# jontio/JAERO

Hardware: AMD Instinct MI355X
Metric: Msamples/s of real 48 kHz PCM through the 10.5 kbps OQPSK demodulator hot path (higher is better)
Workload: dtype f64; 1 GPU; 65536-channel-per-GPU synthetic 48 kHz 10.5 kbps OQPSK continuous (BASELINE configs[2] shape, scaled to 65536 channels per GPU = one wavefront of 64 channels per SIMD), 4096-sample writes, coarse 2^14 FFT every 4096 samples, AFC off, EbNo meters on, Eb/N0 10.0 dB, per-channel carrier (8000 +- 100 Hz), bits, noise, symbol phase; 42 untimed pre-roll steps (the last 18 resident and back to back with ; channels_per_gpu=65536, total_channels=65536, chunk=4096, ebno_meters=True, preroll_steps=42, timing_phases=32, hbm_bytes_per_resident_channel=2256640, resident_channels_max=137027, ranks=1, control_plane=none (single rank), sustain_steps=18

## Files before the change

jaero_amd/csrc/k_burst_front.h:

```cpp
#pragma once
#include "burst_device.h"
#include "jaero_device.h"
#include "k_coarse2.h"
#include "k_coarse6.h"
#include "k_pre8400.h"

#define BLDF(f) (p.S[(size_t)(f) * nchp + ch])
#define BLDI(f) (p.I[(size_t)(f) * nchp + ch])

__device__ __forceinline__ size_t hb_idx(int slot, int nchp, int ch) { return ((size_t)(slot >> 2) * nchp + ch) * 4 + (slot & 3); }
__global__ __launch_bounds__(PF_THREADS) void k_hilbert_fft(const BGeom g, const BPtrs p, int ns, long long n0)
{
    extern __shared__ double hf_xch[];
    const int tid = threadIdx.x, c = tid & 3, T = tid >> 2;
    const int nchp = g.nchp, H = g.hist_len;
    const int cha = blockIdx.x * 8 + 2 * c;
    const long long m0 = ((n0 >> 11) + blockIdx.y) << 11;
    const int i0 = (int)(m0 - n0);
    const int16_t *__restrict__ hist = p.pcmhist;
    CV<16> d;
    {
        const long long tb = m0 - g.hil_lat - 2048 + T + 4LL * H;
#pragma unroll
        for (int s = 0; s < 16; s++)
        {
            const int slot = (int)((tb + 256 * s) % H);
            const size_t o = hb_idx(slot, nchp, cha);
            d.r[s] = (double)hist[o];
            d.i[s] = (double)hist[o + 4];
        }
    }
    pf_fft4096(d, hf_xch, p.tw12, T, c);
    {
        const double2 *__restrict__ Hh = p.hilH + T;
#pragma unroll
        for (int s = 0; s < 16; s++)
        {
            const double2 h = Hh[256 * s];
            const double yr = d.r[s] * h.x - d.i[s] * h.y, yi = d.r[s] * h.y + d.i[s] * h.x;
            d.r[s] = yr; d.i[s] = -yi;
        }
    }
    pf_fft4096(d, hf_xch, p.tw12, T, c);
    const int grp = cha >> 6, lane = cha & 63;
#pragma unroll
    for (int s = 8; s < 16; s++)
    {
        const int i = i0 + T + 256 * (s - 8);
        if (i >= 0 && i < ns)
        {
            const size_t q = ((size_t)grp * g.maxseg + i) * 64 + lane;
            *(double2 *)(p.him + q) = make_double2(d.r[s] / 32768.0, (-d.i[s]) / 32768.0);
        }
    }
}

__global__ void k_hist_push_frames(const int16_t *__restrict__ src, int stride, int nch, int16_t *__restrict__ hist, int nchp, int H,
                                   int slot0, int n)
{
    const int c = blockIdx.x * blockDim.x + threadIdx.x;
    const int i = blockIdx.y;
    if (c >= nchp || i >= n) return;
    int slot = slot0 + i; if (slot >= H) slot -= H;
    hist[hb_idx(slot, nchp, c)] = (c < nch) ? src[(size_t)i * stride + c] : (int16_t)0;
}
__global__ void k_hist_push_chmajor(const int16_t *__restrict__ src, int nch, int n, int16_t *__restrict__ hist, int nchp, int H, int slot0)
{
    __shared__ int16_t tile[64][65];
    const int c0 = blockIdx.x * 64, i0 = blockIdx.y * 64;
    const int tx = threadIdx.x & 63, ty = threadIdx.x >> 6;
    for (int r = ty; r < 64; r += 4)
    {
        const int c = c0 + r, i = i0 + tx;
        tile[r][tx] = (c < nch && i < n) ? src[(size_t)c * n + i] : (int16_t)0;
    }
    __syncthreads();
    for (int r = ty; r < 64; r += 4)
    {
        const int i = i0 + r, c = c0 + tx;
        if (i < n && c < nchp)
        {
            int slot = (slot0 + i) % H;
            hist[hb_idx(slot, nchp, c)] = tile[tx][r];
        }
    }
}

#define FB 8
__device__ __forceinline__ int bwrap(int s, int len) { return s >= len ? s - len : s; }
__device__ __forceinline__ int bback(int s, int lag, int len) { s -= lag; return s < 0 ? s + len : s; }

template <bool HOLD>
__global__ __launch_bounds__(64) void k_burst_front(const BGeom g, const BPtrs p, int n, long long n0)
{
    const int lane = threadIdx.x, grp = blockIdx.x, ch = grp * 64 + lane, nchp = g.nchp;
    double agc_sum = BLDF(BS_AGC_SUM), ma1_re = BLDF(BS_MA1_RE), ma1_im = BLDF(BS_MA1_IM), mav1_sum = BLDF(BS_MAV1_SUM), lastdy = BLDF(BS_LASTDY);
    int cntdown = BLDI(BI_CNTDOWN), maxposcd = BLDI(BI_MAXPOSCD), tri_ptr = BLDI(BI_TRI_PTR);
    const int flags = BLDI(BI_FLAGS);
    int ev_pos = -1, ev_cnt = BLDI(BI_EV_CNT);
    int hold = HOLD ? BLDI(BI_BT_HOLD) : 0;
    const bool trace = (g.flags & 8u) != 0;

    const double *__restrict__ him = p.him + (size_t)grp * g.maxseg * 64 + lane;
    const int16_t *__restrict__ hist = p.pcmhist;
    const int s_re0 = (int)((n0 - g.hil_lat - 1024 + 4LL * g.hist_len) % g.hist_len);
    double *agc_ring = p.agc_ring + (size_t)grp * g.agc_len * 64 + lane;
    double *cvre = p.cvre + (size_t)grp * g.cv_len * 64 + lane;
    double *cvim = p.cvim + (size_t)grp * g.cv_len * 64 + lane;
    double *ma1r = p.ma1re + (size_t)grp * g.ma1_len * 64 + lane;
    double *ma1i = p.ma1im + (size_t)grp * g.ma1_len * 64 + lane;
    double *mav1 = p.mav1 + (size_t)grp * g.mav1_len * 64 + lane;
    double *fa = p.fa + (size_t)grp * g.fa_len * 64 + lane;
    double *bt = p.bt + (size_t)grp * g.bt_len * 64 + lane;

    int s_agc = (int)(n0 % g.agc_len), s_cv = (int)(n0 % g.cv_len), s_ma1 = (int)(n0 % g.ma1_len), s_mav1 = (int)(n0 % g.mav1_len);
    int s_fa = (int)(n0 % g.fa_len), s_bt = (int)(n0 % g.bt_len);
    const double agc_len_d = (double)g.agc_len, ma1_len_d = (double)g.ma1_len, mav1_len_d = (double)g.mav1_len;
    const double btw = g.bt_w, btwc = 1.0 - g.bt_w, faw = g.fa_w, fawc = 1.0 - g.fa_w;
    const int twoPL = 2 * g.PL;

    for (int i0 = 0; i0 < n; i0 += FB)
    {
        double x_re[FB], x_im[FB], o_agc[FB], o_m1r[FB], o_m1i[FB], o_mav[FB], fa_old[FB], fa_new[FB], bt_2[FB], bt_1[FB];
        double co_r[FB], co_i[FB], cn_r[FB], cn_i[FB];
#pragma unroll
        for (int k = 0; k < FB; k++)
        {
            const int ii = (i0 + k < n) ? i0 + k : n - 1;
            const int d = ii - i0;
            x_re[k] = -(((double)hist[hb_idx(bwrap(s_re0 + ii, g.hist_len), nchp, ch)]) / 32768.0); x_im[k] = him[(size_t)ii * 64];
            o_agc[k] = agc_ring[(size_t)bwrap(s_agc + d, g.agc_len) * 64];
            o_m1r[k] = ma1r[(size_t)bwrap(s_ma1 + d, g.ma1_len) * 64];
            o_m1i[k] = ma1i[(size_t)bwrap(s_ma1 + d, g.ma1_len) * 64];
            o_mav[k] = mav1[(size_t)bwrap(s_mav1 + d, g.mav1_len) * 64];
            const int cs = bwrap(s_cv + d, g.cv_len);
            const int c_old = bback(cs, g.bt_lag, g.cv_len), c_new = bwrap(c_old + 1, g.cv_len);
            co_r[k] = cvre[(size_t)c_old * 64]; co_i[k] = cvim[(size_t)c_old * 64];
            cn_r[k] = cvre[(size_t)c_new * 64]; cn_i[k] = cvim[(size_t)c_new * 64];
            const int fs = bwrap(s_fa + d, g.fa_len);
            const int f_old = bback(fs, g.fa_lag, g.fa_len), f_new = bwrap(f_old + 1, g.fa_len);
            fa_old[k] = fa[(size_t)f_old * 64]; fa_new[k] = fa[(size_t)f_new * 64];
            const int bs = bwrap(s_bt + d, g.bt_len);
            bt_2[k] = bt[(size_t)bback(bs, twoPL, g.bt_len) * 64];
            bt_1[k] = bt[(size_t)bback(bs, g.PL, g.bt_len) * 64];
        }
#pragma unroll
        for (int k = 0; k < FB; k++)
        {
            const int i = i0 + k;
            if (i >= n) break;
            const double a = hypot(x_re[k], x_im[k]);
            agc_sum = agc_sum - o_agc[k];
            agc_sum = agc_sum + fabs(a);
            agc_ring[(size_t)s_agc * 64] = fabs(a);
            double gain = 1.414213562 / fmax(agc_sum / agc_len_d, 0.000001);
            gain = fmax(gain, 0.000001);
            const double c_re = x_re[k] * gain, c_im = x_im[k] * gain;
            cvre[(size_t)s_cv * 64] = c_re; cvim[(size_t)s_cv * 64] = c_im;
            double nr = cn_r[k], ni = cn_i[k], orr = co_r[k], oi = co_i[k];
            if (g.bt_lag == 1) { nr = c_re; ni = c_im; }
            if (HOLD)
            {
                if (hold > 0) { orr = 0.0; oi = 0.0; }
                if (hold > 1) { nr = 0.0; ni = 0.0; }
                if (hold > 0) hold--;
            }
            const double dl_re = btw * nr + btwc * orr, dl_im = btw * ni + btwc * oi;
            const double pr = c_re * dl_re - c_im * (-dl_im), pi = c_re * (-dl_im) + c_im * dl_re;
            ma1_re = ma1_re - o_m1r[k]; ma1_im = ma1_im - o_m1i[k];
            ma1_re = ma1_re + pr; ma1_im = ma1_im + pi;
            ma1r[(size_t)s_ma1 * 64] = pr; ma1i[(size_t)s_ma1 * 64] = pi;
            double fastarm = hypot(ma1_re / ma1_len_d, ma1_im / ma1_len_d);
            mav1_sum = mav1_sum - o_mav[k];
            mav1_sum = mav1_sum + fastarm;
            mav1[(size_t)s_mav1 * 64] = fastarm;
            fastarm = mav1_sum / mav1_len_d;
            fa[(size_t)s_fa * 64] = fastarm;
            fastarm -= (faw * fa_new[k] + fawc * fa_old[k]);
            if (fastarm < 0) fastarm = 0;
            double bt_sig = fastarm * fastarm;
            if (bt_sig > 500) bt_sig = 500;
            bt[(size_t)s_bt * 64] = bt_sig;
            const double dy = bt_sig - bt_2[k];
            const double vald = bt_1[k];
            const bool trig = (!cntdown) && (vald > g.pd_thr) && (lastdy >= 0 && dy < 0);
            unsigned long long tm = __ballot(trig);
            if (tm)
            {
                const int pos0 = bback(s_bt, twoPL, g.bt_len);
                const double *btg = p.bt + (size_t)grp * g.bt_len * 64;
                __builtin_amdgcn_fence(__ATOMIC_RELEASE, "wavefront");
                __builtin_amdgcn_s_waitcnt(0x0f70);
                while (tm)
                {
                    const int src = __ffsll((long long)tm) - 1;
                    tm &= tm - 1;
                    double bv = 0.0;
                    int bq = -1;
                    for (int q = lane; q <= twoPL; q += 64)
                    {
                        const double v = btg[(size_t)bwrap(pos0 + q, g.bt_len) * 64 + src];
                        if (bq < 0 || v > bv) { bv = v; bq = q; }
                    }
#pragma unroll
                    for (int off = 32; off > 0; off >>= 1)
                    {
                        const double ov = __shfl_xor(bv, off, 64);
                        const int oq = __shfl_xor(bq, off, 64);
                        if (oq >= 0 && (bq < 0 || ov > bv || (ov == bv && oq < bq))) { bv = ov; bq = oq; }
                    }
                    if (lane == src) { cntdown = twoPL; maxposcd = bq; }
                }
            }
            if (cntdown > 0) cntdown--;
            lastdy = dy;
            bool fire = false;
            if (!maxposcd) { maxposcd--; fire = true; }
            else if (maxposcd > 0) maxposcd--;
            if (fire)
            {
                tri_ptr = 0;
                if (trace && ev_cnt < g.ev_cap)
                {
                    double *e = p.evlog + ((size_t)ch * g.ev_cap + ev_cnt) * 3;
                    e[0] = (double)(n0 + i); e[1] = BEV_PEAK; e[2] = 0; ev_cnt++;
                }
            }
            if (tri_ptr < g.tri_sz) tri_ptr++;
            else if (tri_ptr == g.tri_sz) { tri_ptr++; ev_pos = i; }
            s_agc = bwrap(s_agc + 1, g.agc_len); s_cv = bwrap(s_cv + 1, g.cv_len); s_ma1 = bwrap(s_ma1 + 1, g.ma1_len);
            s_mav1 = bwrap(s_mav1 + 1, g.mav1_len); s_fa = bwrap(s_fa + 1, g.fa_len); s_bt = bwrap(s_bt + 1, g.bt_len);
        }
    }
    BLDF(BS_AGC_SUM) = agc_sum; BLDF(BS_MA1_RE) = ma1_re; BLDF(BS_MA1_IM) = ma1_im; BLDF(BS_MAV1_SUM) = mav1_sum; BLDF(BS_LASTDY) = lastdy;
    BLDI(BI_CNTDOWN) = cntdown; BLDI(BI_MAXPOSCD) = maxposcd; BLDI(BI_TRI_PTR) = tri_ptr; BLDI(BI_EV_POS) = ev_pos; BLDI(BI_EV_CNT) = ev_cnt;
    (void)flags;
    if (HOLD) BLDI(BI_BT_HOLD) = hold;
    const unsigned long long em = __ballot(ev_pos >= 0 && ch < g.nch);
    if (lane == 0) p.ev_mask[grp] = em;
}

__global__ __launch_bounds__(1024) void k_ev_compact(const unsigned long long *__restrict__ mask, int ngroups, int *__restrict__ ev_list, int *__restrict__ ev_count)
{
    __shared__ int part[1024];
    const int t = threadIdx.x;
    const int per = (ngroups + 1023) / 1024;
    const int g0 = t * per, g1 = (g0 + per < ngroups) ? g0 + per : ngroups;
    int cnt = 0;
    for (int gq = g0; gq < g1; gq++) cnt += __popcll(mask[gq]);
    part[t] = cnt;
    __syncthreads();
    for (int off = 1; off < 1024; off <<= 1)
    {
        const int v = (t >= off) ? part[t - off] : 0;
        __syncthreads();
        part[t] += v;
        __syncthreads();
    }
    int base = part[t] - cnt;
    for (int gq = g0; gq < g1; gq++)
    {
        unsigned long long m = mask[gq];
        while (m)
        {
            const int ln = __ffsll((long long)m) - 1;
            m &= m - 1;
            ev_list[base++] = gq * 64 + ln;
        }
    }
    if (t == 1023) *ev_count = part[1023];
}

#define TRI_N 32768
#define TRI_H 16384

template <int NTHREADS>
__device__ __forceinline__ void tri_argmax_first(double &v, int &idx, double *red_val, int *red_idx, int t)
{
#pragma unroll
    for (int off = 32; off > 0; off >>= 1)
    {
        const double ov = __shfl_xor(v, off, 64);
        const int oi = __shfl_xor(idx, off, 64);
        if (oi >= 0 && (idx < 0 || ov > v || (ov == v && oi < idx))) { v = ov; idx = oi; }
    }
    __syncthreads();
    if ((t & 63) == 0) { red_val[t >> 6] = v; red_idx[t >> 6] = idx; }
    __syncthreads();
    v = red_val[0]; idx = red_idx[0];
#pragma unroll
    for (int w = 1; w < NTHREADS / 64; w++)
    {
        const double ov = red_val[w];
        const int oi = red_idx[w];
        if (oi >= 0 && (idx < 0 || ov > v || (ov == v && oi < idx))) { v = ov; idx = oi; }
    }
}

#define TRI_THREADS 256
#define TRI_XCH C6_XCH13
template <bool oq>
__global__ __launch_bounds__(TRI_THREADS, 2) void k_trident(const BGeom g, const BPtrs p, long long n0)
{
    extern __shared__ __attribute__((aligned(16))) double xch[];
    __shared__ double red_val[TRI_THREADS / 64];
    __shared__ int red_idx[TRI_THREADS / 64];
    __shared__ double sh_bb[2];
    double *dl = xch;
    const int t = threadIdx.x, nchp = g.nchp;
    const int nev = *p.ev_count;
    const double hzperbin = g.Fs / ((double)TRI_N);
    const int b = jd_qround((0.25 * g.fb) / hzperbin), b4 = b >> 2;
    const int psb = jd_qround((0.5 * g.fb) / hzperbin);
    const int nx = gridDim.x < 8 ? 1 : 8;
    const int xcd = blockIdx.x % nx, wx = blockIdx.x / nx, nwx = (gridDim.x + nx - 1 - xcd) / nx;
    const int e_lo = (int)(((long long)nev * xcd) / nx), e_hi = (int)(((long long)nev * (xcd + 1)) / nx);
    for (int li = e_lo + wx; li < e_hi; li += nwx)
    {
        const int ch = p.ev_list[li];
        const int grp = ch >> 6, lane = ch & 63;
        const int evp = p.I[(size_t)BI_EV_POS * nchp + ch];
        const long long w0 = n0 + evp - g.tri_sz - g.D1 + 8LL * g.cv_len;
        const double *__restrict__ cvre = p.cvre + (size_t)grp * g.cv_len * 64 + lane;
        double mag[16];
        double bv = -1.0, bre = 0.0, bim = 0.0;
        int bi = -1;
        double minval = 0.0;
        int minvalbin = 0;
        double mv = 0.0; int mi = -1;
        double lv = 0.0; int lidx = -1;
        double hv = 0.0; int hidx = -1;
        for (int pass = 0; pass < 8; pass++)
        {
            const int which = oq ? (pass & 1) : (pass >> 2), r = oq ? (pass >> 1) : (pass & 3);
            const int off = which ? g.nb : 0, len = which ? g.nt : g.nb;
            if (!oq && pass == 4)
            {
                minval = bv; minvalbin = bi;
                tri_argmax_first<TRI_THREADS>(minval, minvalbin, red_val, red_idx, t);
                if (bi == minvalbin) { sh_bb[0] = bre; sh_bb[1] = bim; }
                if (!(minval > 0.0)) minvalbin = 0;
            }
            CV<32> d;
            const int slot0 = (int)((w0 + off) % g.cv_len);
#pragma unroll
            for (int s = 0; s < 32; s++)
            {
                const int n = s * TRI_THREADS + t;
                if (s * TRI_THREADS >= len) { d.r[s] = 0.0; d.i[s] = 0.0; continue; }
                double x0 = 0.0, x1 = 0.0;
                if (n < len)
                {
                    int sl = slot0 + n; if (sl >= g.cv_len) sl -= g.cv_len;
                    x0 = cvre[(size_t)sl * 64];
                }
                if (len > 8192 && n + 8192 < len)
                {
                    int sl = slot0 + n + 8192; while (sl >= g.cv_len) sl -= g.cv_len;
                    x1 = cvre[(size_t)sl * 64];
                }
                double fr = x0, fi = 0.0;
                if (r == 0) fr += x1; else if (r == 1) fi -= x1; else if (r == 2) fr -= x1; else fi += x1;
                if (r == 0) { d.r[s] = fr; d.i[s] = fi; }
                else
                {
                    const int m = n * r;
                    double2 w = p.tw15[m & (TRI_H - 1)];
                    if (m & TRI_H) { w.x = -w.x; w.y = -w.y; }
                    d.r[s] = fr * w.x - fi * w.y; d.i[s] = fr * w.y + fi * w.x;
                }
            }
            wg_fft13_e32(d, xch, p.tw14, t);
            if (which == 0)
            {
#pragma unroll
                for (int s = 0; s < 16; s++)
                {
                    const int k = 4 * (s * TRI_THREADS + t) + r;
                    const double a = hypot(d.r[s], d.i[s]);
                    mag[s] = a;
                    if (a > bv || (a == bv && k < bi)) { bv = a; bi = k; bre = d.r[s]; bim = d.i[s]; }
                }
            }
            else if (oq)
            {
                __syncthreads();
#pragma unroll
                for (int s = 0; s < 16; s++) dl[s * TRI_THREADS + t] = hypot(d.r[s], d.i[s]) - mag[s];
                __syncthreads();
                for (int q = b4 + t; q < (TRI_H >> 2) - b4; q += TRI_THREADS)
                {
                    const double tv = dl[q - b4] + dl[q + b4] - dl[q];
                    const int k = 4 * q + r;
                    if (mi < 0 || tv > mv || (tv == mv && k < mi)) { mv = tv; mi = k; }
                }
            }
            else
            {
#pragma unroll
                for (int s = 0; s < 16; s++)
                {
                    const int k = 4 * (s * TRI_THREADS + t) + r;
                    if (k > 50)
                    {
                        const double a = hypot(d.r[s], d.i[s]);
                        if ((k < minvalbin - (psb / 2)) && (a > lv || (a == lv && lidx >= 0 && k < lidx))) { lv = a; lidx = k; }
                        if ((k > minvalbin + (psb / 2)) && (a > hv || (a == hv && hidx >= 0 && k < hidx))) { hv = a; hidx = k; }
                    }
                }
            }
        }
        TriResult res;
        res.pad = 0;
        if (oq)
        {
            minval = bv; minvalbin = bi;
            tri_argmax_first<TRI_THREADS>(minval, minvalbin, red_val, red_idx, t);
            if (bi == minvalbin) { sh_bb[0] = bre; sh_bb[1] = bim; }
            if (!(minval > 0.0)) minvalbin = 0;
            tri_argmax_first<TRI_THREADS>(mv, mi, red_val, red_idx, t);
            const double maxval = mv;
            const int maxvalbin = mi;
            res.ok = (maxval > 500.0) && (fabs((((double)(maxvalbin - minvalbin))) * hzperbin) < 20.0);
            const double bbx = (minval > 0.0) ? sh_bb[0] : 0.0, bby = (minval > 0.0) ? sh_bb[1] : 0.0;
            const double carrierphase = atan2(bby, bbx) - (M_PI / 4.0);
            res.freq = hzperbin * (double)minvalbin;
            res.phase_deg = (180.0 / M_PI) * carrierphase;
            res.vol_gain = 1.4142 * 500.0 / minval;
            res.metric = maxval;
        }
        else
        {
            tri_argmax_first<TRI_THREADS>(lv, lidx, red_val, red_idx, t);
            const int maxtoppos = (lidx >= 0) ? lidx : 0;
            tri_argmax_first<TRI_THREADS>(hv, hidx, red_val, red_idx, t);
            const int maxtopposhigh = (hidx >= 0) ? hidx : 0;
            const int distfrompeak = abs(maxtoppos - minvalbin);
            res.ok = (minval > 500.0) && (abs(distfrompeak - psb) < abs(psb / 20));
            const double bbx = (minval > 0.0) ? sh_bb[0] : 0.0, bby = (minval > 0.0) ? sh_bb[1] : 0.0;
            const double carrierphase = atan2(bby, bbx) - (M_PI / 4.0);
            res.freq = ((double)((maxtopposhigh + maxtoppos) / 2)) * hzperbin;
            res.phase_deg = (180.0 / M_PI) * carrierphase;
            res.vol_gain = 1.4142 * (500.0 / (minval / 3));
            res.metric = minval;
        }
        if (t == 0) p.tri[ch] = res;
        __syncthreads();
    }
}
```

jaero_amd/csrc/k_coarse6.h:

```cpp
#pragma once
#include "k_coarse2.h"

#ifndef C4_TABN
#define C4_TABN 3584
#endif
#define C6_FENCE __builtin_amdgcn_sched_barrier(0)
__device__ __forceinline__ double2 c6_sq(const double2 a)
{
#pragma clang fp contract(fast)
    return make_double2(a.x * a.x - a.y * a.y, 2.0 * (a.x * a.y));
}

#ifndef C6_TRACE
#define C6_TRACE(i)
#endif

template <int CTRL, int ROWMASK>
__device__ __forceinline__ void c6_argmax_step(double &bv, int &bi)
{
    const int lo = __builtin_amdgcn_update_dpp(__double2loint(bv), __double2loint(bv), CTRL, ROWMASK, 0xf, false);
    const int hi = __builtin_amdgcn_update_dpp(__double2hiint(bv), __double2hiint(bv), CTRL, ROWMASK, 0xf, false);
    const int oi = __builtin_amdgcn_update_dpp(bi, bi, CTRL, ROWMASK, 0xf, false);
    const double ov = __hiloint2double(hi, lo);
    const bool take = (oi >= 0) & ((bi < 0) | (ov > bv) | ((ov == bv) & (oi < bi)));
    bv = take ? ov : bv;
    bi = take ? oi : bi;
}
__device__ __forceinline__ void c6_wave_argmax(double &bv, int &bi)
{
    c6_argmax_step<0xB1, 0xf>(bv, bi);
    c6_argmax_step<0x4E, 0xf>(bv, bi);
    c6_argmax_step<0x141, 0xf>(bv, bi);
    c6_argmax_step<0x140, 0xf>(bv, bi);
    c6_argmax_step<0x142, 0xa>(bv, bi);
    c6_argmax_step<0x143, 0xc>(bv, bi);
    bv = __hiloint2double(__builtin_amdgcn_readlane(__double2hiint(bv), 63), __builtin_amdgcn_readlane(__double2loint(bv), 63));
    bi = __builtin_amdgcn_readlane(bi, 63);
}

#define C6_XCH 16448

__device__ __forceinline__ constexpr int c6_k(int s) { return s < 16 ? 2 * s : 2 * (s - 16) + 1; }

__device__ __forceinline__ void c6_fft32(CV<32> &x)
{
#pragma clang fp contract(fast)
#pragma unroll
    for (int j = 0; j < 16; j++)
    {
        const double ar = x.r[j], ai = x.i[j], br = x.r[j + 16], bi = x.i[j + 16];
        x.r[j] = ar + br; x.i[j] = ai + bi;
        double dr = ar - br, di = ai - bi;
        cmul_w64(dr, di, 2 * j);
        x.r[j + 16] = dr; x.i[j + 16] = di;
    }
    C6_FENCE;
#pragma unroll
    for (int h = 0; h < 2; h++)
    {
        CV<16> in, out;
#pragma unroll
        for (int j = 0; j < 16; j++) { in.r[j] = x.r[16 * h + j]; in.i[j] = x.i[16 * h + j]; }
        regfft<16>(in, out);
#pragma unroll
        for (int j = 0; j < 16; j++) { x.r[16 * h + j] = out.r[j]; x.i[16 * h + j] = out.i[j]; }
        C6_FENCE;
    }
}

__device__ __forceinline__ void c6_twiddle32(CV<32> &x, const double2 p1)
{
#pragma clang fp contract(fast)
    auto app = [&](int slot, const double2 w) __attribute__((always_inline)) {
        const double r = x.r[slot] * w.x - x.i[slot] * w.y, i = x.r[slot] * w.y + x.i[slot] * w.x;
        x.r[slot] = r; x.i[slot] = i;
    };
    const double2 p2 = c6_sq(p1);
    double2 e = p2;
    app(16, p1);
#pragma unroll
    for (int j = 1; j < 16; j++)
    {
        app(j, e);
        app(16 + j, cmul2(e, p1));
        if (j < 15) e = cmul2(e, p2);
    }
}

__device__ __forceinline__ void wg_fft14_e32(CV<32> &d, double *xch, const double2 *__restrict__ tw, int t)
{
#pragma clang fp contract(fast)
    const double2 st1 = tw[t], st2 = tw[32 * (t & 15)];
    const int k1u = t >> 4, n3 = t & 15, odd = k1u & 1;
    const int e1w0 = t, e1w1 = (t + 16) & 511;
    const int e1r = k1u * 512 + odd * 16 + n3;
    const int e1rw = e1r + 496 - 512 * odd;
    const int e2w = k1u + n3 * 513;
    const int e2r = t;

    c6_fft32(d);
    c6_twiddle32(d, st1);
    C6_FENCE;
    jd_lds_barrier();
#pragma unroll
    for (int s = 0; s < 32; s++) xch[c6_k(s) * 512 + ((c6_k(s) & 1) ? e1w1 : e1w0)] = d.r[s];
    jd_lds_barrier();
#pragma unroll
    for (int m = 0; m < 32; m++) d.r[m] = xch[(m < 31 ? e1r + 16 * m : e1rw)];
    jd_lds_barrier();
#pragma unroll
    for (int s = 0; s < 32; s++) xch[c6_k(s) * 512 + ((c6_k(s) & 1) ? e1w1 : e1w0)] = d.i[s];
    jd_lds_barrier();
#pragma unroll
    for (int m = 0; m < 32; m++) d.i[m] = xch[(m < 31 ? e1r + 16 * m : e1rw)];
    C6_FENCE;
    c6_fft32(d);
    c6_twiddle32(d, st2);
    C6_FENCE;
    jd_lds_barrier();
#pragma unroll
    for (int s = 0; s < 32; s++) xch[e2w + (c6_k(s) & 15) * 32 + (c6_k(s) >> 4) * 8208] = d.r[s];
    jd_lds_barrier();
#pragma unroll
    for (int m = 0; m < 32; m++) d.r[m] = xch[e2r + (m & 15) * 513 + (m >> 4) * 8208];
    jd_lds_barrier();
#pragma unroll
    for (int s = 0; s < 32; s++) xch[e2w + (c6_k(s) & 15) * 32 + (c6_k(s) >> 4) * 8208] = d.i[s];
    jd_lds_barrier();
#pragma unroll
    for (int m = 0; m < 32; m++) d.i[m] = xch[e2r + (m & 15) * 513 + (m >> 4) * 8208];
    C6_FENCE;
    {
        CV<16> in, o0, o1;
#pragma unroll
        for (int j = 0; j < 16; j++) { in.r[j] = d.r[j]; in.i[j] = d.i[j]; }
        regfft<16>(in, o0);
        C6_FENCE;
#pragma unroll
        for (int j = 0; j < 16; j++) { in.r[j] = d.r[16 + j]; in.i[j] = d.i[16 + j]; }
        regfft<16>(in, o1);
#pragma unroll
        for (int k3 = 0; k3 < 16; k3++) { d.r[2 * k3] = o0.r[k3]; d.i[2 * k3] = o0.i[k3]; d.r[2 * k3 + 1] = o1.r[k3]; d.i[2 * k3 + 1] = o1.i[k3]; }
    }
}


#define C6_XCH13 8208
__device__ __forceinline__ void wg_fft13_e32(CV<32> &d, double *xch, const double2 *__restrict__ tw, int t)
{
#pragma clang fp contract(fast)
    const double2 st1 = tw[t], st2 = tw[32 * (t & 15)];
    const int k1a = t >> 4, n3 = t & 15;
    const int e1r = k1a * 256 + n3;
    const int e2w = k1a + 513 * n3;
    c6_fft32(d);
    c6_twiddle32(d, st1);
    C6_FENCE;
    jd_lds_barrier();
#pragma unroll
    for (int s = 0; s < 32; s++) (xch + c6_k(s) * 256)[t] = d.r[s];
    jd_lds_barrier();
#pragma unroll
    for (int m = 0; m < 32; m++) d.r[m] = (xch + (m >> 4) * 4096 + (m & 15) * 16)[e1r];
    jd_lds_barrier();
#pragma unroll
    for (int s = 0; s < 32; s++) (xch + c6_k(s) * 256)[t] = d.i[s];
    jd_lds_barrier();
#pragma unroll
    for (int m = 0; m < 32; m++) d.i[m] = (xch + (m >> 4) * 4096 + (m & 15) * 16)[e1r];
    C6_FENCE;
#pragma unroll
    for (int g2 = 0; g2 < 2; g2++)
    {
        CV<16> in, out;
#pragma unroll
        for (int j = 0; j < 16; j++) { in.r[j] = d.r[16 * g2 + j]; in.i[j] = d.i[16 * g2 + j]; }
        regfft<16>(in, out);
        c4_twiddle16(out, st2);
#pragma unroll
        for (int j = 0; j < 16; j++) { d.r[16 * g2 + j] = out.r[j]; d.i[16 * g2 + j] = out.i[j]; }
        C6_FENCE;
    }
    jd_lds_barrier();
#pragma unroll
    for (int s = 0; s < 32; s++) (xch + (s >> 4) * 16 + (s & 15) * 32)[e2w] = d.r[s];
    jd_lds_barrier();
#pragma unroll
    for (int m = 0; m < 32; m++) d.r[m] = (xch + (m >> 4) * 256 + (m & 15) * 513)[t];
    jd_lds_barrier();
#pragma unroll
    for (int s = 0; s < 32; s++) (xch + (s >> 4) * 16 + (s & 15) * 32)[e2w] = d.i[s];
    jd_lds_barrier();
#pragma unroll
    for (int m = 0; m < 32; m++) d.i[m] = (xch + (m >> 4) * 256 + (m & 15) * 513)[t];
    C6_FENCE;
    {
        CV<16> in, o0, o1;
#pragma unroll
        for (int j = 0; j < 16; j++) { in.r[j] = d.r[j]; in.i[j] = d.i[j]; }
        regfft<16>(in, o0);
        C6_FENCE;
#pragma unroll
        for (int j = 0; j < 16; j++) { in.r[j] = d.r[16 + j]; in.i[j] = d.i[16 + j]; }
        regfft<16>(in, o1);
#pragma unroll
        for (int k3 = 0; k3 < 16; k3++) { d.r[2 * k3] = o0.r[k3]; d.i[2 * k3] = o0.i[k3]; d.r[2 * k3 + 1] = o1.r[k3]; d.i[2 * k3 + 1] = o1.i[k3]; }
    }
}

template <int LOG2N>
__device__ __forceinline__ void c6_fft(CV<32> &d, double *xch, const double2 *__restrict__ tw, int t)
{
    int tt = t;
    asm volatile("" : "+v"(tt));
    if constexpr (LOG2N == 14) wg_fft14_e32(d, xch, tw, tt);
    else wg_fft13_e32(d, xch, tw, tt);
}

__device__ __noinline__ void c6_build_window(double *wt, int startbin, int t, int nthreads)
{
    for (int i = t; i <= startbin + 1; i += nthreads)
    {
        const double c = cos(M_PI_2 * ((double)i) / ((double)startbin));
        wt[i] = (i == 0) ? 1.0 : ((i <= startbin) ? c * c : 0.0);
    }
}

template <bool W8400, int LOG2N = 14>
__device__ __forceinline__ void coarse6_body(const JGeom g, const JPtrs p, const int *__restrict__ chan_list, int nlist, const double2 *__restrict__ tw)
{
    constexpr int N = 1 << LOG2N;
    constexpr int E = 32;
    constexpr int NT = N / E;
    constexpr int XCH = LOG2N == 14 ? C6_XCH : C6_XCH13;
    extern __shared__ __attribute__((aligned(16))) double xch[];
    __shared__ double red_val[NT / 64];
    __shared__ int red_idx[NT / 64];
    const int t0 = threadIdx.x;
    const int nchp = g.nchp;
    int tab_startbin = -1;

    CV<E> d;
    int ch_next = ((int)blockIdx.x < nlist) ? (chan_list ? jd_sload(chan_list + blockIdx.x) : (int)blockIdx.x) : 0;
    int bp_next = jd_sload(p.I + (size_t)I_BB_PTR * nchp + ch_next);
    for (int li = blockIdx.x; li < nlist; li += gridDim.x)
    {
        int t = t0;
        asm volatile("" : "+v"(t));
        const int ch = ch_next, bb_ptr = bp_next;
        const double2 *__restrict__ ring = p.bbring + (size_t)ch * N;
        const int ln = li + (int)gridDim.x;
        const bool has_next = ln < nlist;
        if (has_next)
        {
            ch_next = chan_list ? jd_sload(chan_list + ln) : ln;
            bp_next = jd_sload(p.I + (size_t)I_BB_PTR * nchp + ch_next);
        }
        const double lockingbw = jd_sload(p.S + (size_t)S_LOCKINGBW * nchp + ch);
        double fs_l = g.Fs;
        asm volatile("" : "+s"(fs_l));
        int startbin, expectedpeakbin;
        {
            const double hzperbin = fs_l * (1.0 / ((double)N));
            startbin = __builtin_amdgcn_readfirstlane((int)fmax(round(lockingbw / hzperbin), 1.0));
            expectedpeakbin = __builtin_amdgcn_readfirstlane((int)round(g.fb / (2.0 * hzperbin)));
        }
        const int stopbin = N - startbin;
        double *__restrict__ y = p.y + (size_t)ch * N;

        if (li == (int)blockIdx.x)
        {
#pragma unroll
            for (int s = 0; s < E; s++)
            {
                const double2 v = ring[(bb_ptr + s * NT + t) & (N - 1)];
                d.r[s] = v.x; d.i[s] = v.y;
            }
        }
        C6_TRACE(0);
        c6_fft<LOG2N>(d, xch, tw, t);
        C6_TRACE(1);
        if constexpr (W8400)
        {
            const bool persistent = startbin < C4_TABN - 1;
            double *wt = persistent ? xch + XCH : xch;
            if (!persistent || startbin != tab_startbin)
            {
                jd_lds_barrier();
                c6_build_window(wt, startbin, t, NT);
                jd_lds_barrier();
                if (persistent) tab_startbin = startbin;
            }
#pragma unroll
            for (int s0 = 0; s0 < E; s0 += 8)
            {
#pragma unroll
                for (int s = s0; s < s0 + 8; s++)
                {
                    const int k = s * NT + t;
                    const int i = (k <= N / 2) ? k : N - k;
                    const double w = wt[i <= startbin ? i : startbin + 1];
                    const double re = d.r[s] * w, im = d.i[s] * w;
                    d.r[s] = im; d.i[s] = re;
                }
                C6_FENCE;
            }
            if (!persistent) jd_lds_barrier();
        }
        else
        {
#pragma unroll
            for (int s = 0; s < E; s++)
            {
                const int k = s * NT + t;
                const bool z = (k >= startbin) && (k <= stopbin);
                const double re = z ? 0.0 : d.r[s], im = z ? 0.0 : d.i[s];
                d.r[s] = im; d.i[s] = re;
            }
        }
        c6_fft<LOG2N>(d, xch, tw, t);
        C6_TRACE(2);
#pragma unroll
        for (int s = 0; s < E; s++)
        {
            const double re = d.i[s], im = d.r[s];
            d.r[s] = re * re - im * im;
            d.i[s] = re * im + im * re;
        }
        c6_fft<LOG2N>(d, xch, tw, t);
        C6_TRACE(3);
        jd_lds_barrier();
        CoarseSlotState cst;
        {
            double yv[E];
#pragma unroll
            for (int s = 0; s < E; s++) d.r[s] = d.r[s] * d.r[s] + d.i[s] * d.i[s];
            C6_FENCE;
#pragma unroll
            for (int s = 0; s < E; s++) yv[s] = __builtin_nontemporal_load((y + ((s * NT) ^ (N / 2))) + t);
            C6_FENCE;
            cst = coarse_slot_load_v(g, p, ch);
            int bpn = bp_next, chn = ch_next, tp = t;
            asm volatile("" : "+v"(bpn), "+v"(chn), "+v"(tp));
            typedef double c6_v2 __attribute__((ext_vector_type(2)));
            const c6_v2 *__restrict__ ringn = (const c6_v2 *)(p.bbring + (size_t)chn * N);
            const int toffp = bpn + tp;
#pragma unroll
            for (int s = 0; s < E; s++)
            {
                const int ib = (s * NT) ^ (N / 2);
                const double yn = yv[s] * 0.9 + 0.5 * jd_log10(fmax(d.r[s], 1.0));
                __builtin_nontemporal_store(yn, (y + ib) + t);
                (xch + ib)[t] = yn;
                {
                    const c6_v2 v = __builtin_nontemporal_load(ringn + ((toffp + s * NT) & (N - 1)));
                    d.r[s] = v.x; d.i[s] = v.y;
                }
                if ((s & 3) == 3) C6_FENCE;
            }
            C6_TRACE(4);
            jd_lds_barrier();
            C6_TRACE(5);
        }
        C6_TRACE(6);
        double fs_e = g.Fs;
        asm volatile("" : "+s"(fs_e));
        const double hzperbin = fs_e * (1.0 / ((double)N));
        const int i0 = __builtin_amdgcn_readfirstlane((int)round((-lockingbw / hzperbin) + ((double)(N / 2))));
        const int i1 = __builtin_amdgcn_readfirstlane((int)round((lockingbw / hzperbin) + ((double)(N / 2))));
        double best = 0;
        int besti = -1;
        const bool fold_inside = (i0 - expectedpeakbin - 1 >= 0) && (i1 + expectedpeakbin < N) && (i0 >= 0);
        if (fold_inside)
        {
            const int nblk = (i1 - i0 + 4 * NT - 1) / (4 * NT);
            for (int b = 0; b < nblk; b++)
            {
                double val[4];
#pragma unroll
                for (int u = 0; u < 4; u++)
                {
                    const int i = i0 + t + (4 * b + u) * NT;
                    const int ic = i < i1 ? i : i1 - 1;
                    const double *lo = xch + (ic - expectedpeakbin), *hi = xch + (ic + expectedpeakbin);
                    double v = 0;
                    v += (lo[1] + hi[-1]);
                    v += (lo[0] + hi[0]);
                    v += (lo[-1] + hi[1]);
                    val[u] = v;
                }
#pragma unroll
                for (int u = 0; u < 4; u++)
                {
                    const int i = i0 + t + (4 * b + u) * NT;
                    const bool take = (i < i1) & (val[u] > best);
                    best = take ? val[u] : best;
                    besti = take ? i : besti;
                }
            }
        }
        else
        {
            for (int i = i0 + t; i < i1; i += NT)
            {
                if ((i < 0) || (i >= N)) continue;
                double val = 0;
                for (int j = -1; j <= 1; j++)
                {
                    if (((i - expectedpeakbin - j) < 0) || ((i + expectedpeakbin + j) >= N)) continue;
                    val += (xch[i - expectedpeakbin - j] + xch[i + expectedpeakbin + j]);
                }
                if (val > best) { best = val; besti = i; }
            }
        }
        C6_TRACE(7);
        int bigchange;
        {
            double bv = best;
            int bi = besti;
            c6_wave_argmax(bv, bi);
            if ((t & 63) == 0) { red_val[t >> 6] = bv; red_idx[t >> 6] = bi; }
            C6_TRACE(8);
            jd_lds_barrier();
            bv = red_val[0]; bi = red_idx[0];
#pragma unroll
            for (int w = 1; w < NT / 64; w++)
            {
                const double ov = red_val[w];
                const int oi = red_idx[w];
                const bool take = (oi >= 0) & ((bi < 0) | (ov > bv) | ((ov == bv) & (oi < bi)));
                bv = take ? ov : bv;
                bi = take ? oi : bi;
            }
            bigchange = coarse_slot_apply(g, p, ch, cst, (bi >= 0) ? bi : (N / 2), N, hzperbin, lockingbw, t == 0);
            C6_TRACE(9);
        }
        if (bigchange)
        {
            __syncthreads();
            double2 *ringw = p.bbring + (size_t)ch * N;
            for (int i = t; i < N; i += NT) { y[i] = 20; ringw[i] = make_double2(0.0, 0.0); }
        }
        C6_TRACE(10);
    }
}

__global__ __launch_bounds__(C2_THREADS) void k_coarse6(const JGeom g, const JPtrs p, const int *__restrict__ chan_list,
                                                           int nlist, const double2 *__restrict__ tw)
{
    coarse6_body<false>(g, p, chan_list, nlist, tw);
}
__global__ __launch_bounds__(C2_THREADS) void k_coarse6_w8400(const JGeom g, const JPtrs p, const int *__restrict__ chan_list,
                                                                 int nlist, const double2 *__restrict__ tw)
{
    coarse6_body<true>(g, p, chan_list, nlist, tw);
}
__global__ __launch_bounds__(256, 2) void k_coarse6_13(const JGeom g, const JPtrs p, const int *__restrict__ chan_list,
                                                        int nlist, const double2 *__restrict__ tw)
{
    coarse6_body<false, 13>(g, p, chan_list, nlist, tw);
}
```

Baseline: 11800 Msamples/s.

## Absorb inter-pass FFT twiddles into radix-2 butterfly roots of later passes

Adds a templated path, on by default through C6_ABSORB=2, in the 2^13/2^14 workgroup FFTs. Instead of separate twiddle multiplies after each pass, the twiddle is folded into the butterfly roots of the next register FFT. That pass uses a bit-reversed FMA radix-2 form driven by repeated squaring of the twiddle ratio. LDS write indices are permuted to match the bit-reversed output. This removes the per-element twiddle complex multiplies, but the radix-2 form may need more flops than the tuned regfft/radix-32 kernels, and the squaring chain can add rounding error. The burst-front call site keeps the old non-absorbed variant explicitly.

```diff
diff --git a/jaero_amd/csrc/k_burst_front.h b/jaero_amd/csrc/k_burst_front.h
--- a/jaero_amd/csrc/k_burst_front.h
+++ b/jaero_amd/csrc/k_burst_front.h
@@ -370,7 +370,7 @@
                     d.r[s] = fr * w.x - fi * w.y; d.i[s] = fr * w.y + fi * w.x;
                 }
             }
-            wg_fft13_e32(d, xch, p.tw14, t);
+            wg_fft13_e32<0>(d, xch, p.tw14, t);
             if (which == 0)
             {
 #pragma unroll
diff --git a/jaero_amd/csrc/k_coarse6.h b/jaero_amd/csrc/k_coarse6.h
--- a/jaero_amd/csrc/k_coarse6.h
+++ b/jaero_amd/csrc/k_coarse6.h
@@ -87,19 +87,138 @@
     }
 }
 
+#ifndef C6_ABSORB
+#define C6_ABSORB 2
+#endif
+
+__device__ __forceinline__ constexpr int c6_brev(int v, int bits)
+{
+    int r = 0;
+    for (int i = 0; i < bits; i++) r |= ((v >> i) & 1) << (bits - 1 - i);
+    return r;
+}
+
+__device__ __forceinline__ double2 c6_root_mul(const double2 p, int idx)
+{
+#pragma clang fp contract(fast)
+    const int e = idx & 15;
+    double2 r = p;
+    if (e != 0)
+    {
+        const double wr = jd_w64r(e), wi = jd_w64i(e);
+        r = make_double2(p.x * wr - p.y * wi, p.x * wi + p.y * wr);
+    }
+    return (idx & 16) ? make_double2(r.y, -r.x) : r;
+}
+
+__device__ __forceinline__ void c6_ratio_powers(const double2 r, double2 (&P)[5])
+{
+    P[0] = r;
+#pragma unroll
+    for (int i = 1; i < 5; i++) P[i] = c6_sq(P[i - 1]);
+}
+
+template <int L, int OFF, int Z>
+__device__ __forceinline__ void c6_afft(CV<32> &x, const double2 (&P)[5])
+{
+    constexpr int LG = L == 32 ? 5 : 4, S = 64 / L;
+#pragma unroll
+    for (int lv = 0; lv < LG; lv++)
+    {
+#pragma unroll
+        for (int b = 0; b < (1 << lv); b++)
+        {
+            const int half = L >> (lv + 1);
+            const double2 w = c6_root_mul(P[LG - 1 - lv], half * (S * c6_brev(b, lv) + Z));
+#pragma unroll
+            for (int j = 0; j < half; j++)
+            {
+                const int ia = OFF + 2 * half * b + j, ib = ia + half;
+                const double ar = x.r[ia], ai = x.i[ia], br = x.r[ib], bi = x.i[ib];
+                const double ur = __builtin_fma(-w.y, bi, __builtin_fma(w.x, br, ar));
+                const double ui = __builtin_fma(w.x, bi, __builtin_fma(w.y, br, ai));
+                x.r[ia] = ur; x.i[ia] = ui;
+                x.r[ib] = __builtin_fma(2.0, ar, -ur); x.i[ib] = __builtin_fma(2.0, ai, -ui);
+            }
+        }
+        C6_FENCE;
+    }
+}
+
+__device__ __forceinline__ void c6_afft16x2(CV<32> &x, const double2 r)
+{
+    double2 P[5];
+    c6_ratio_powers(r, P);
+    c6_afft<16, 0, 0>(x, P);
+    c6_afft<16, 16, 2>(x, P);
+}
+
+template <int L, int OFF>
+__device__ __forceinline__ void c6_twiddle_brev(CV<32> &x, const double2 c, const double2 s)
+{
+#pragma clang fp contract(fast)
+    constexpr int LG = L == 32 ? 5 : 4;
+    auto app = [&](int slot, const double2 w) __attribute__((always_inline)) {
+        const double r = x.r[slot] * w.x - x.i[slot] * w.y, i = x.r[slot] * w.y + x.i[slot] * w.x;
+        x.r[slot] = r; x.i[slot] = i;
+    };
+    const double2 s2 = c6_sq(s);
+    double2 e = c;
+#pragma unroll
+    for (int j = 0; j < L / 2; j++)
+    {
+        app(OFF + c6_brev(2 * j, LG), e);
+        app(OFF + c6_brev(2 * j + 1, LG), cmul2(e, s));
+        if (j < L / 2 - 1) e = cmul2(e, s2);
+    }
+}
+
+template <bool ABSORBED>
+__device__ __forceinline__ void c6_pass3(CV<32> &d, const double2 r)
+{
+    if constexpr (ABSORBED)
+    {
+        c6_afft16x2(d, r);
+        const CV<32> o = d;
+#pragma unroll
+        for (int k3 = 0; k3 < 16; k3++)
+        {
+            d.r[2 * k3] = o.r[c6_brev(k3, 4)]; d.i[2 * k3] = o.i[c6_brev(k3, 4)];
+            d.r[2 * k3 + 1] = o.r[16 + c6_brev(k3, 4)]; d.i[2 * k3 + 1] = o.i[16 + c6_brev(k3, 4)];
+        }
+    }
+    else
+    {
+        CV<16> in, o0, o1;
+#pragma unroll
+        for (int j = 0; j < 16; j++) { in.r[j] = d.r[j]; in.i[j] = d.i[j]; }
+        regfft<16>(in, o0);
+        C6_FENCE;
+#pragma unroll
+        for (int j = 0; j < 16; j++) { in.r[j] = d.r[16 + j]; in.i[j] = d.i[16 + j]; }
+        regfft<16>(in, o1);
+#pragma unroll
+        for (int k3 = 0; k3 < 16; k3++) { d.r[2 * k3] = o0.r[k3]; d.i[2 * k3] = o0.i[k3]; d.r[2 * k3 + 1] = o1.r[k3]; d.i[2 * k3 + 1] = o1.i[k3]; }
+    }
+}
+
+template <int AB = C6_ABSORB>
 __device__ __forceinline__ void wg_fft14_e32(CV<32> &d, double *xch, const double2 *__restrict__ tw, int t)
 {
 #pragma clang fp contract(fast)
-    const double2 st1 = tw[t], st2 = tw[32 * (t & 15)];
     const int k1u = t >> 4, n3 = t & 15, odd = k1u & 1;
+    const double2 st1 = tw[AB ? 16 * k1u : t], st2 = tw[AB == 2 ? t : 32 * n3];
+    double2 st3 = st2;
+    if constexpr (AB == 1) st3 = tw[k1u * n3];
     const int e1w0 = t, e1w1 = (t + 16) & 511;
     const int e1r = k1u * 512 + odd * 16 + n3;
     const int e1rw = e1r + 496 - 512 * odd;
     const int e2w = k1u + n3 * 513;
     const int e2r = t;
+    auto k2of = [](int s) __attribute__((always_inline)) { return AB ? c6_brev(s, 5) : c6_k(s); };
 
     c6_fft32(d);
-    c6_twiddle32(d, st1);
+    if constexpr (AB == 0) c6_twiddle32(d, st1);
     C6_FENCE;
     jd_lds_barrier();
 #pragma unroll
@@ -114,47 +233,48 @@
 #pragma unroll
     for (int m = 0; m < 32; m++) d.i[m] = xch[(m < 31 ? e1r + 16 * m : e1rw)];
     C6_FENCE;
-    c6_fft32(d);
-    c6_twiddle32(d, st2);
-    C6_FENCE;
-    jd_lds_barrier();
-#pragma unroll
-    for (int s = 0; s < 32; s++) xch[e2w + (c6_k(s) & 15) * 32 + (c6_k(s) >> 4) * 8208] = d.r[s];
+    if constexpr (AB == 0)
+    {
+        c6_fft32(d);
+        c6_twiddle32(d, st2);
+    }
+    else
+    {
+        double2 P[5];
+        c6_ratio_powers(st1, P);
+        c6_afft<32, 0, 0>(d, P);
+        if constexpr (AB == 1) c6_twiddle_brev<32, 0>(d, st3, st2);
+    }
+    C6_FENCE;
+    jd_lds_barrier();
+#pragma unroll
+    for (int s = 0; s < 32; s++) xch[e2w + (k2of(s) & 15) * 32 + (k2of(s) >> 4) * 8208] = d.r[s];
     jd_lds_barrier();
 #pragma unroll
     for (int m = 0; m < 32; m++) d.r[m] = xch[e2r + (m & 15) * 513 + (m >> 4) * 8208];
     jd_lds_barrier();
 #pragma unroll
-    for (int s = 0; s < 32; s++) xch[e2w + (c6_k(s) & 15) * 32 + (c6_k(s) >> 4) * 8208] = d.i[s];
+    for (int s = 0; s < 32; s++) xch[e2w + (k2of(s) & 15) * 32 + (k2of(s) >> 4) * 8208] = d.i[s];
     jd_lds_barrier();
 #pragma unroll
     for (int m = 0; m < 32; m++) d.i[m] = xch[e2r + (m & 15) * 513 + (m >> 4) * 8208];
     C6_FENCE;
-    {
-        CV<16> in, o0, o1;
-#pragma unroll
-        for (int j = 0; j < 16; j++) { in.r[j] = d.r[j]; in.i[j] = d.i[j]; }
-        regfft<16>(in, o0);
-        C6_FENCE;
-#pragma unroll
-        for (int j = 0; j < 16; j++) { in.r[j] = d.r[16 + j]; in.i[j] = d.i[16 + j]; }
-        regfft<16>(in, o1);
-#pragma unroll
-        for (int k3 = 0; k3 < 16; k3++) { d.r[2 * k3] = o0.r[k3]; d.i[2 * k3] = o0.i[k3]; d.r[2 * k3 + 1] = o1.r[k3]; d.i[2 * k3 + 1] = o1.i[k3]; }
-    }
+    c6_pass3<AB == 2>(d, st2);
 }
 
 
 #define C6_XCH13 8208
+template <int AB = C6_ABSORB>
 __device__ __forceinline__ void wg_fft13_e32(CV<32> &d, double *xch, const double2 *__restrict__ tw, int t)
 {
 #pragma clang fp contract(fast)
-    const double2 st1 = tw[t], st2 = tw[32 * (t & 15)];
     const int k1a = t >> 4, n3 = t & 15;
+    const double2 st1 = tw[AB ? 16 * k1a : t], st2 = tw[AB == 2 ? t : 32 * n3];
     const int e1r = k1a * 256 + n3;
     const int e2w = k1a + 513 * n3;
+    auto k2of = [](int s) __attribute__((always_inline)) { return AB ? c6_brev(s & 15, 4) : (s & 15); };
     c6_fft32(d);
-    c6_twiddle32(d, st1);
+    if constexpr (AB == 0) c6_twiddle32(d, st1);
     C6_FENCE;
     jd_lds_barrier();
 #pragma unroll
@@ -169,43 +289,45 @@
 #pragma unroll
     for (int m = 0; m < 32; m++) d.i[m] = (xch + (m >> 4) * 4096 + (m & 15) * 16)[e1r];
     C6_FENCE;
-#pragma unroll
-    for (int g2 = 0; g2 < 2; g2++)
-    {
-        CV<16> in, out;
-#pragma unroll
-        for (int j = 0; j < 16; j++) { in.r[j] = d.r[16 * g2 + j]; in.i[j] = d.i[16 * g2 + j]; }
-        regfft<16>(in, out);
-        c4_twiddle16(out, st2);
-#pragma unroll
-        for (int j = 0; j < 16; j++) { d.r[16 * g2 + j] = out.r[j]; d.i[16 * g2 + j] = out.i[j]; }
+    if constexpr (AB == 0)
+    {
+#pragma unroll
+        for (int g2 = 0; g2 < 2; g2++)
+        {
+            CV<16> in, out;
+#pragma unroll
+            for (int j = 0; j < 16; j++) { in.r[j] = d.r[16 * g2 + j]; in.i[j] = d.i[16 * g2 + j]; }
+            regfft<16>(in, out);
+            c4_twiddle16(out, st2);
+#pragma unroll
+            for (int j = 0; j < 16; j++) { d.r[16 * g2 + j] = out.r[j]; d.i[16 * g2 + j] = out.i[j]; }
+            C6_FENCE;
+        }
+    }
+    else
+    {
+        c6_afft16x2(d, st1);
+        if constexpr (AB == 1)
+        {
+            c6_twiddle_brev<16, 0>(d, tw[n3 * k1a], st2);
+            c6_twiddle_brev<16, 16>(d, tw[n3 * (k1a + 16)], st2);
+        }
         C6_FENCE;
     }
     jd_lds_barrier();
 #pragma unroll
-    for (int s = 0; s < 32; s++) (xch + (s >> 4) * 16 + (s & 15) * 32)[e2w] = d.r[s];
+    for (int s = 0; s < 32; s++) (xch + (s >> 4) * 16 + k2of(s) * 32)[e2w] = d.r[s];
     jd_lds_barrier();
 #pragma unroll
     for (int m = 0; m < 32; m++) d.r[m] = (xch + (m >> 4) * 256 + (m & 15) * 513)[t];
     jd_lds_barrier();
 #pragma unroll
-    for (int s = 0; s < 32; s++) (xch + (s >> 4) * 16 + (s & 15) * 32)[e2w] = d.i[s];
+    for (int s = 0; s < 32; s++) (xch + (s >> 4) * 16 + k2of(s) * 32)[e2w] = d.i[s];
     jd_lds_barrier();
 #pragma unroll
     for (int m = 0; m < 32; m++) d.i[m] = (xch + (m >> 4) * 256 + (m & 15) * 513)[t];
     C6_FENCE;
-    {
-        CV<16> in, o0, o1;
-#pragma unroll
-        for (int j = 0; j < 16; j++) { in.r[j] = d.r[j]; in.i[j] = d.i[j]; }
-        regfft<16>(in, o0);
-        C6_FENCE;
-#pragma unroll
-        for (int j = 0; j < 16; j++) { in.r[j] = d.r[16 + j]; in.i[j] = d.i[16 + j]; }
-        regfft<16>(in, o1);
-#pragma unroll
-        for (int k3 = 0; k3 < 16; k3++) { d.r[2 * k3] = o0.r[k3]; d.i[2 * k3] = o0.i[k3]; d.r[2 * k3 + 1] = o1.r[k3]; d.i[2 * k3 + 1] = o1.i[k3]; }
-    }
+    c6_pass3<AB == 2>(d, st2);
 }
 
 template <int LOG2N>
```

Result: faster. 12090 Msamples/s, median of 6 (+2.4%).
